# leggedrobotics/delora

Measured on AMD Instinct MI355X. Metric: training scan-pairs/sec, KITTI 64x2048 range images, higher is better.
Workload: dtype f32; 1 GPU; KITTI-shaped 64x2048, batch=8 pairs/GPU, raw scans of ~141k points (ragged, raster order), steps rotate over 8 distinct HBM-resident batches, online normals, ResNet pose CNN (11.9M params, identity-pretrained state), Adam; BASELINE configs[1]; global_batch=8, parallelism=dp1, cnn=fp32, cnn_impl=hip trunk: fp32 MFMA, fused Winograd F(2x2,3x3) + direct implicit GEMM, channels_last=False, hip_graph=False, distinct_batches=8, priming_steps=8

## Files before the change

### delora_amd/csrc/wino_conv_body.h

```cpp
  constexpr int DEAD = STR == 1 ? 3 : (STR == 2 ? 0 : -1);
  constexpr int TR = WN_TILES / TC;
  constexpr int RH = 2 * TR + 2, RW = 2 * TC + 2;
  constexpr int NPIX = RH * RW, NRI = (NPIX + 31) / 32;
  constexpr int RAWBUF = NRI * 256;
  constexpr int NR_IT = (NRI + 7) / 8;
  constexpr int BUF = 2 * 16 * WN_PLANE;
  static_assert((2 * BUF + 2 * RAWBUF) * 4 <= 163840, "LDS budget");
  __shared__ __attribute__((aligned(16))) float lds[2 * BUF + 2 * RAWBUF];
  float* rawbase = lds + 2 * BUF;
#define WN_BUFOF(CH) (lds + (((CH) + 1) & 1) * BUF)

  const int tid = threadIdx.x, lane = tid & 63, wave = __builtin_amdgcn_readfirstlane(tid >> 6);
  const int li = lane & 31, half = lane >> 5;
  const int mb = wave & 1, nb = (wave >> 1) & 1, xh = wave >> 2;
  const int KT = a.K / WN_KB;
  const int tiles_w = RAG ? ((a.W + 1) / 2 + TC - 1) / TC : (a.W / 2) / TC;
  const int tiles_h = RAG ? ((a.H + 1) / 2 + TR - 1) / TR : (a.H / 2) / TR;
  const int nsplit = SPLIT ? a.splits : 1;
  const int ngroups = a.N * tiles_h * tiles_w * KT * nsplit;
  const int nchunks = a.C / WN_CK / nsplit;

  const int tb = wave & 3, tc4 = lane & 1, ttile = (wave >> 2) * 32 + (lane >> 1);
  const int ttr = ttile / TC, ttc = ttile % TC;
  const int j0 = tb == 0 ? 0 : (tb == 2 ? 2 : 1), j1 = tb == 2 ? 1 : (tb == 3 ? 3 : 2);
  const float sgn_s = tb == 1 ? 1.f : -1.f;
  const f32x2 sgn = {sgn_s, sgn_s};
  const int t_wr = tb * WN_PLANE + ttile * 8 + ((tc4 ^ ((ttile >> 3) & 1)) * 4);
  const int t_rd = ((2 * ttr) * RW + 2 * ttc) * 8 + tc4 * 4;
  constexpr int NRAW_W = (NRI + 1) / 2;
  const unsigned lane16 = 16u * (unsigned)lane;
  const int arow = mb * 32 + li, brow = nb * 32 + li;
  const int a_off = arow * 8 + ((half ^ ((arow >> 3) & 1)) * 4);
  const int b_off = 16 * WN_PLANE + brow * 8 + ((half ^ ((brow >> 3) & 1)) * 4);

  int n, k0, gh, gw;
  int cb = 0;
  float* ysp = a.y;
  const float* xn;
  int rowmask[4];
  bool edge;
  unsigned raw_g[NR_IT];
#define WN_SETUP(G, LN)                                                                                                   \
  {                                                                                                                       \
    int t_ = wn_xcd_swizzle((G), ngroups);                                                                                \
    if (SPLIT) { cb = (t_ % nsplit) * nchunks; t_ /= nsplit; }        \
    const int kt_ = t_ % KT; t_ /= KT;                                                                                    \
    gw = t_ % tiles_w; t_ /= tiles_w;                                                                                     \
    gh = t_ % tiles_h;                                                                                                    \
    n = t_ / tiles_h;                                                                                                     \
    k0 = kt_ * WN_KB;                                                                                                     \
    const int h_base_ = gh * TR * 2 - 1, w_base_ = gw * TC * 2 - 1;                       \
    xn = a.x + (size_t)n * a.H * a.W * a.C;                                                                               \
    _Pragma("unroll") for (int i = 0; i < 4; ++i) {                                                                       \
      const int h_ = h_base_ + 2 * ttr + i;                                                                               \
      rowmask[i] = (h_ >= 0 && h_ < a.H) ? -1 : 0;                                                                        \
    }                                                                                                                     \
    edge = __builtin_amdgcn_readfirstlane((int)(h_base_ < 0 || h_base_ + RH > a.H)) != 0;                                                                           \
    _Pragma("unroll") for (int it = 0; it < NR_IT; ++it) {                                                                \
      const int p_ = min(min(2 * wave + it, NRI - 1) * 32 + ((LN) >> 1), NPIX - 1);         \
      int h_ = h_base_ + p_ / RW;                                                                                         \
      h_ = h_ < 0 ? 0 : (h_ >= a.H ? a.H - 1 : h_);                                                                       \
      int w_ = w_base_ + p_ % RW;                                                                                         \
      if (RAG) { w_ %= a.W; w_ = w_ < 0 ? w_ + a.W : w_; }        \
      else w_ = w_ < 0 ? w_ + a.W : (w_ >= a.W ? w_ - a.W : w_);                                                           \
      raw_g[it] = 4u * (unsigned)((h_ * a.W + w_) * a.C + ((LN) & 1) * 4);                                       \
    }                                                                                                                     \
  }

  const unsigned lds_base = (unsigned)(__SIZE_TYPE__)((__attribute__((address_space(3))) char*)lds);
  const int m0_raw = __builtin_amdgcn_readfirstlane((int)(lds_base + 4u * (unsigned)(2 * BUF + min(2 * wave, NRI - 1) * 256)));
  const int m0_u = __builtin_amdgcn_readfirstlane((int)(lds_base + 4u * (unsigned)(16 * WN_PLANE + 2 * wave * WN_PLANE)));
#define WN_RAW_ALL(CH)                                                                                                    \
  {                                                                                                                       \
    const float* rp_ = xn + ((CH) + cb) * WN_CK;                                                                          \
    const int m_ = m0_raw + ((CH) & 1) * (RAWBUF * 4);                                                                    \
    if (2 * wave + 1 < NRI)                                                                                               \
      asm volatile("s_mov_b32 m0, %0\n\ts_nop 0\n\tglobal_load_lds_dwordx4 %1, %3\n\tglobal_load_lds_dwordx4 %2, %4 offset:1024"     \
                   :: "s"(m_), "v"(raw_g[0]), "v"(raw_g[NR_IT - 1]), "s"(rp_), "s"(rp_ - 256) : "memory");                  \
    else if (2 * wave < NRI)                                                                                              \
      asm volatile("s_mov_b32 m0, %0\n\ts_nop 0\n\tglobal_load_lds_dwordx4 %1, %2" :: "s"(m_), "v"(raw_g[0]), "s"(rp_) : "memory");  \
  }
#define WN_U_ALL(CH, BUFP)                                                                                                \
  {                                                                                                                       \
    const float* up_ = a.u + (((size_t)((CH) + cb) * KT + (k0 >> 6)) * 16 + 2 * wave) * 512;                               \
    const int m_ = m0_u + (int)((BUFP) - lds) * 4;                                                                        \
    if (DEAD == 3 && (wave & 1))                                                 \
      asm volatile("s_mov_b32 m0, %0\n\ts_nop 0\n\tglobal_load_lds_dwordx4 %1, %2\n\tglobal_load_lds_dwordx4 %1, %2 offset:1024" \
                   :: "s"(m_), "v"(lane16), "s"(up_) : "memory");                                                         \
    else if (DEAD == 0 && !(wave & 1))                                                           \
      asm volatile("s_mov_b32 m0, %0\n\ts_nop 0\n\tglobal_load_lds_dwordx4 %1, %2 offset:2112\n\tglobal_load_lds_dwordx4 %1, %2 offset:3136" \
                   :: "s"(m_), "v"(lane16), "s"(up_ - 16) : "memory");                                                    \
    else                                                                                                                  \
    asm volatile("s_mov_b32 m0, %0\n\ts_nop 0\n\tglobal_load_lds_dwordx4 %1, %2\n\tglobal_load_lds_dwordx4 %1, %2 offset:1024\n\t" \
                 "global_load_lds_dwordx4 %1, %3 offset:2112\n\tglobal_load_lds_dwordx4 %1, %3 offset:3136"                \
                 :: "s"(m_), "v"(lane16), "s"(up_), "s"(up_ - 16) : "memory");                                            \
  }
#define WN_TROW_LD(I, RB)                                                                                                 \
  {                                                                                                                       \
    dd[(I) & 1][0] = *reinterpret_cast<const i32x4*>((RB) + t_rd + ((I) * RW + j0) * 8);                                  \
    dd[(I) & 1][1] = *reinterpret_cast<const i32x4*>((RB) + t_rd + ((I) * RW + j1) * 8);                                  \
  }
#define WN_TROW_FIN(I)                                                                                                    \
  {                                                                                                                       \
    if (edge) { asm volatile("" ::: "memory"); dd[(I) & 1][0] &= rowmask[I]; dd[(I) & 1][1] &= rowmask[I]; }      \
    const f32x4 da_ = __builtin_bit_cast(f32x4, dd[(I) & 1][0]), db_ = __builtin_bit_cast(f32x4, dd[(I) & 1][1]);         \
    asm volatile("v_pk_fma_f32 %0, %1, %2, %3" : "=v"(tt[I][0]) : "v"(__builtin_shufflevector(db_, db_, 0, 1)), "s"(sgn), "v"(__builtin_shufflevector(da_, da_, 0, 1))); \
    asm volatile("v_pk_fma_f32 %0, %1, %2, %3" : "=v"(tt[I][1]) : "v"(__builtin_shufflevector(db_, db_, 2, 3)), "s"(sgn), "v"(__builtin_shufflevector(da_, da_, 2, 3))); \
  }
#define WN_TROW(I, RB) WN_TROW_LD(I, RB) WN_TROW_FIN(I)
#define WN_PK_ADD(X, Y) ({ f32x2 l_, h_;                                                                                    \
    asm volatile("v_pk_add_f32 %0, %1, %2" : "=v"(l_) : "v"((X)[0]), "v"((Y)[0]));                                        \
    asm volatile("v_pk_add_f32 %0, %1, %2" : "=v"(h_) : "v"((X)[1]), "v"((Y)[1]));                                        \
    __builtin_shufflevector(l_, h_, 0, 1, 2, 3); })
#define WN_PK_SUB(X, Y) ({ f32x2 l_, h_;                                                                                    \
    asm volatile("v_pk_add_f32 %0, %1, %2 neg_lo:[0,1] neg_hi:[0,1]" : "=v"(l_) : "v"((X)[0]), "v"((Y)[0]));              \
    asm volatile("v_pk_add_f32 %0, %1, %2 neg_lo:[0,1] neg_hi:[0,1]" : "=v"(h_) : "v"((X)[1]), "v"((Y)[1]));              \
    __builtin_shufflevector(l_, h_, 0, 1, 2, 3); })
#define WN_V0()                                                                                                           \
  {                                                                                                                       \
    f32x2 tt[4][2];                                                                                                       \
    i32x4 dd[2][2];                                                                                                       \
    const float* rb_ = rawbase;                                                                                           \
    float* vb_ = WN_BUFOF(0) + t_wr;                                                                                      \
    WN_TROW(0, rb_) WN_TROW(1, rb_) WN_TROW(2, rb_) WN_TROW(3, rb_)                                                       \
    *reinterpret_cast<f32x4*>(vb_ + 0 * 4 * WN_PLANE) = WN_PK_SUB(tt[0], tt[2]);                                                    \
    *reinterpret_cast<f32x4*>(vb_ + 1 * 4 * WN_PLANE) = WN_PK_ADD(tt[1], tt[2]);                                                    \
    *reinterpret_cast<f32x4*>(vb_ + 2 * 4 * WN_PLANE) = WN_PK_SUB(tt[2], tt[1]);                                                    \
    *reinterpret_cast<f32x4*>(vb_ + 3 * 4 * WN_PLANE) = WN_PK_SUB(tt[1], tt[3]);                                                    \
  }
#define WN_LOAD_FRAGS_FROM(XL, BP)                                                                                        \
  {                                                                                                                       \
    av[(XL) & 1] = *reinterpret_cast<const f32x4*>((BP) + (xh * 8 + (XL)) * WN_PLANE + a_off);                            \
    bv[(XL) & 1] = *reinterpret_cast<const f32x4*>((BP) + (xh * 8 + (XL)) * WN_PLANE + b_off);                            \
  }
#define WN_LOAD_FRAGS(XL) WN_LOAD_FRAGS_FROM(XL, cur)
#define WN_M(XL, J, ...)                                                                                                  \
  {                                                                                                                       \
    acc[XL] = __builtin_amdgcn_mfma_f32_32x32x2f32(av[(XL) & 1][J], bv[(XL) & 1][J], acc[XL], 0, 0, 0);                   \
    __VA_ARGS__                                                                                                           \
    __builtin_amdgcn_sched_barrier(0);                                                                                    \
  }
#define WN_MZ(XL, J, ...)                                                                                                 \
  {                                                                                                                       \
    acc[XL] = __builtin_amdgcn_mfma_f32_32x32x2f32(av[(XL) & 1][J], bv[(XL) & 1][J], wn_zero16, 0, 0, 0);                 \
    __VA_ARGS__                                                                                                           \
    __builtin_amdgcn_sched_barrier(0);                                                                                    \
  }
#define WN_LOAD_FRAGS_B(XL, B, BP)                                                                                        \
  {                                                                                                                       \
    av[B] = *reinterpret_cast<const f32x4*>((BP) + (xh * 8 + (XL)) * WN_PLANE + a_off);                                   \
    bv[B] = *reinterpret_cast<const f32x4*>((BP) + (xh * 8 + (XL)) * WN_PLANE + b_off);                                   \
  }
#define WN_MB(XL, B, J, ...)                                                                                              \
  {                                                                                                                       \
    acc[XL] = __builtin_amdgcn_mfma_f32_32x32x2f32(av[B][J], bv[B][J], acc[XL], 0, 0, 0);                                 \
    __VA_ARGS__                                                                                                           \
    __builtin_amdgcn_sched_barrier(0);                                                                                    \
  }
#define WN_MZB(XL, B, J, ...)                                                                                             \
  {                                                                                                                       \
    acc[XL] = __builtin_amdgcn_mfma_f32_32x32x2f32(av[B][J], bv[B][J], wn_zero16, 0, 0, 0);                               \
    __VA_ARGS__                                                                                                           \
    __builtin_amdgcn_sched_barrier(0);                                                                                    \
  }

  const f32x16 wn_zero16 = {0.f, 0.f, 0.f, 0.f, 0.f, 0.f, 0.f, 0.f, 0.f, 0.f, 0.f, 0.f, 0.f, 0.f, 0.f, 0.f};
  int grp = blockIdx.x;
  WN_SETUP(grp, lane)
  WN_RAW_ALL(0)
  WN_RAW_ALL(min(1, nchunks - 1))
  WN_U_ALL(0, WN_BUFOF(0))
  asm volatile("s_waitcnt vmcnt(0)" ::: "memory");
  __syncthreads();
  WN_V0()
  for (;;) {
    __syncthreads();
    WN_T(0)
    f32x4 av[2], bv[2];
    f32x2 tt[4][2];
    i32x4 dd[2][2];
    f32x16 acc[8];
    {
      float* cur = WN_BUFOF(0);
      if (DEAD == 0) WN_LOAD_FRAGS_B(1, 0, cur)
      else WN_LOAD_FRAGS(0)
    }
#define WN_CHUNK_BODY(MF)                                                                                                 \
    {                                                                                                                     \
      float* cur = WN_BUFOF(ch);                                                                                          \
      float* nxt = WN_BUFOF(ch + 1);                                                                                      \
      const float* rb = rawbase + ((ch + 1) & 1) * RAWBUF;                                                                \
      float* vb = nxt + t_wr;                                                                                             \
      MF(0, 0, WN_IF_FR(WN_LOAD_FRAGS(1))) WN_M(0, 1, WN_IF_U(WN_U_ALL(ch + 1, nxt)))                                     \
      WN_M(0, 2, )                                                                                                        \
                            \
      WN_M(0, 3, WN_IF_RAW(if (ch + 2 < nchunks) WN_RAW_ALL(ch + 2)))                                                     \
       \
      MF(1, 0, WN_IF_FR(WN_LOAD_FRAGS(2))) WN_M(1, 1, WN_IF_T(WN_TROW_LD(0, rb) WN_TROW_LD(1, rb))) WN_M(1, 2, ) WN_M(1, 3, WN_IF_T(WN_TROW_FIN(0) WN_TROW_FIN(1))) \
      MF(2, 0, WN_IF_FR(WN_LOAD_FRAGS(3))) WN_M(2, 1, WN_IF_T(WN_TROW_LD(2, rb) WN_TROW_LD(3, rb))) WN_M(2, 2, ) WN_M(2, 3, WN_IF_T(WN_TROW_FIN(2) WN_TROW_FIN(3))) \
      MF(3, 0, WN_IF_FR(WN_LOAD_FRAGS(4)) WN_IF_T(*reinterpret_cast<f32x4*>(vb + 0 * 4 * WN_PLANE) = WN_PK_SUB(tt[0], tt[2]);))   \
      WN_M(3, 1, WN_IF_T(*reinterpret_cast<f32x4*>(vb + 1 * 4 * WN_PLANE) = WN_PK_ADD(tt[1], tt[2]);)) WN_M(3, 2, ) WN_M(3, 3, ) \
      MF(4, 0, WN_IF_FR(WN_LOAD_FRAGS(5)) WN_IF_T(*reinterpret_cast<f32x4*>(vb + 2 * 4 * WN_PLANE) = WN_PK_SUB(tt[2], tt[1]);))   \
      WN_M(4, 1, WN_IF_T(*reinterpret_cast<f32x4*>(vb + 3 * 4 * WN_PLANE) = WN_PK_SUB(tt[1], tt[3]);)) WN_M(4, 2, ) WN_M(4, 3, ) \
      MF(5, 0, WN_IF_FR(WN_LOAD_FRAGS(6))) WN_M(5, 1, ) WN_M(5, 2, ) WN_M(5, 3, )                                         \
      MF(6, 0, WN_IF_FR(WN_LOAD_FRAGS(7))) WN_M(6, 1, ) WN_M(6, 2, ) WN_M(6, 3, )                                         \
      asm volatile("s_waitcnt vmcnt(0) lgkmcnt(0)" ::: "memory");                                                         \
      WN_IF_BAR(__builtin_amdgcn_s_barrier();)                                                                            \
      __builtin_amdgcn_sched_barrier(0);                                                                                  \
      MF(7, 0, WN_IF_FR(WN_LOAD_FRAGS_FROM(0, nxt))) WN_M(7, 1, ) WN_M(7, 2, ) WN_M(7, 3, )                               \
    }
#define WN_TAIL_BODY(MF)                                                                                                  \
    {                                                                                                                     \
      float* cur = WN_BUFOF(nchunks - 1);                                                                                 \
      MF(0, 0, WN_LOAD_FRAGS(1)) WN_M(0, 1, ) WN_M(0, 2, ) WN_M(0, 3, )                                                   \
      MF(1, 0, WN_LOAD_FRAGS(2)) WN_M(1, 1, ) WN_M(1, 2, ) WN_M(1, 3, )                                                   \
      MF(2, 0, WN_LOAD_FRAGS(3)) WN_M(2, 1, ) WN_M(2, 2, ) WN_M(2, 3, )                                                   \
      MF(3, 0, WN_LOAD_FRAGS(4)) WN_M(3, 1, ) WN_M(3, 2, ) WN_M(3, 3, )                                                   \
      MF(4, 0, WN_LOAD_FRAGS(5)) WN_M(4, 1, ) WN_M(4, 2, ) WN_M(4, 3, )                                                   \
      MF(5, 0, WN_LOAD_FRAGS(6)) WN_M(5, 1, ) WN_M(5, 2, ) WN_M(5, 3, )                                                   \
      MF(6, 0, WN_LOAD_FRAGS(7)) WN_M(6, 1, ) WN_M(6, 2, ) WN_M(6, 3, )                                                   \
      MF(7, 0, ) WN_M(7, 1, ) WN_M(7, 2, ) WN_M(7, 3, )                                                                   \
    }
#define WN_TX(...) { __VA_ARGS__ }
#define WN_VST(I, EXPR) WN_TX(*reinterpret_cast<f32x4*>(vb + (I) * 4 * WN_PLANE) = EXPR;)
#define WN_CHUNK_BODY_F(MF)                                                                                               \
    {                                                                                                                     \
      float* cur = WN_BUFOF(ch);                                                                                          \
      float* nxt = WN_BUFOF(ch + 1);                                                                                      \
      const float* rb = rawbase + ((ch + 1) & 1) * RAWBUF;                                                                \
      float* vb = nxt + t_wr;                                                                                             \
      MF(0, 0, 0, WN_LOAD_FRAGS_B(1, 1, cur)) WN_MB(0, 0, 1, WN_U_ALL(ch + 1, nxt)) WN_MB(0, 0, 2, )                      \
      WN_MB(0, 0, 3, if (ch + 2 < nchunks) WN_RAW_ALL(ch + 2))                                                            \
      MF(1, 1, 0, WN_LOAD_FRAGS_B(2, 0, cur)) WN_MB(1, 1, 1, WN_TX(WN_TROW_LD(0, rb) WN_TROW_LD(1, rb))) WN_MB(1, 1, 2, ) \
      WN_MB(1, 1, 3, WN_TX(WN_TROW_FIN(0) WN_TROW_FIN(1)))                                                                \
      MF(2, 0, 0, WN_LOAD_FRAGS_B(4, 1, cur)) WN_MB(2, 0, 1, WN_TX(WN_TROW_LD(2, rb) WN_TROW_LD(3, rb))) WN_MB(2, 0, 2, ) \
      WN_MB(2, 0, 3, WN_TX(WN_TROW_FIN(2) WN_TROW_FIN(3)))                                                                \
      MF(4, 1, 0, WN_LOAD_FRAGS_B(5, 0, cur) WN_VST(0, WN_PK_SUB(tt[0], tt[2])))                                          \
      WN_MB(4, 1, 1, WN_VST(1, WN_PK_ADD(tt[1], tt[2]))) WN_MB(4, 1, 2, ) WN_MB(4, 1, 3, )                                \
      MF(5, 0, 0, WN_LOAD_FRAGS_B(6, 1, cur) WN_VST(2, WN_PK_SUB(tt[2], tt[1])))                                          \
      WN_MB(5, 0, 1, WN_VST(3, WN_PK_SUB(tt[1], tt[3]))) WN_MB(5, 0, 2, ) WN_MB(5, 0, 3, )                                \
      asm volatile("s_waitcnt vmcnt(0) lgkmcnt(0)" ::: "memory");                                                         \
      __builtin_amdgcn_s_barrier();                                                                                       \
      __builtin_amdgcn_sched_barrier(0);                                                                                  \
      MF(6, 1, 0, WN_LOAD_FRAGS_B(0, 0, nxt)) WN_MB(6, 1, 1, ) WN_MB(6, 1, 2, ) WN_MB(6, 1, 3, )                          \
    }
#define WN_TAIL_BODY_F(MF)                                                                                                \
    {                                                                                                                     \
      float* cur = WN_BUFOF(nchunks - 1);                                                                                 \
      MF(0, 0, 0, WN_LOAD_FRAGS_B(1, 1, cur)) WN_MB(0, 0, 1, ) WN_MB(0, 0, 2, ) WN_MB(0, 0, 3, )                          \
      MF(1, 1, 0, WN_LOAD_FRAGS_B(2, 0, cur)) WN_MB(1, 1, 1, ) WN_MB(1, 1, 2, ) WN_MB(1, 1, 3, )                          \
      MF(2, 0, 0, WN_LOAD_FRAGS_B(4, 1, cur)) WN_MB(2, 0, 1, ) WN_MB(2, 0, 2, ) WN_MB(2, 0, 3, )                          \
      MF(4, 1, 0, WN_LOAD_FRAGS_B(5, 0, cur)) WN_MB(4, 1, 1, ) WN_MB(4, 1, 2, ) WN_MB(4, 1, 3, )                          \
      MF(5, 0, 0, WN_LOAD_FRAGS_B(6, 1, cur)) WN_MB(5, 0, 1, ) WN_MB(5, 0, 2, ) WN_MB(5, 0, 3, )                          \
      MF(6, 1, 0, ) WN_MB(6, 1, 1, ) WN_MB(6, 1, 2, ) WN_MB(6, 1, 3, )                                                    \
    }
#define WN_CHUNK_BODY_B(MF)                                                                                               \
    {                                                                                                                     \
      float* cur = WN_BUFOF(ch);                                                                                          \
      float* nxt = WN_BUFOF(ch + 1);                                                                                      \
      const float* rb = rawbase + ((ch + 1) & 1) * RAWBUF;                                                                \
      float* vb = nxt + t_wr;                                                                                             \
      MF(1, 0, 0, WN_LOAD_FRAGS_B(2, 1, cur) WN_U_ALL(ch + 1, nxt))                                                       \
      WN_MB(1, 0, 1, WN_TX(WN_TROW_LD(0, rb) WN_TROW_LD(1, rb)))                                                          \
      WN_MB(1, 0, 2, if (ch + 2 < nchunks) WN_RAW_ALL(ch + 2)) WN_MB(1, 0, 3, WN_TX(WN_TROW_FIN(0) WN_TROW_FIN(1)))       \
      MF(2, 1, 0, WN_LOAD_FRAGS_B(3, 0, cur)) WN_MB(2, 1, 1, WN_TX(WN_TROW_LD(2, rb) WN_TROW_LD(3, rb))) WN_MB(2, 1, 2, ) \
      WN_MB(2, 1, 3, WN_TX(WN_TROW_FIN(2) WN_TROW_FIN(3)))                                                                \
      MF(3, 0, 0, WN_LOAD_FRAGS_B(5, 1, cur) WN_VST(0, WN_PK_SUB(tt[0], tt[2])))                                          \
      WN_MB(3, 0, 1, WN_VST(1, WN_PK_ADD(tt[1], tt[2]))) WN_MB(3, 0, 2, ) WN_MB(3, 0, 3, )                                \
      MF(5, 1, 0, WN_LOAD_FRAGS_B(6, 0, cur) WN_VST(2, WN_PK_SUB(tt[2], tt[1])))                                          \
      WN_MB(5, 1, 1, WN_VST(3, WN_PK_SUB(tt[1], tt[3]))) WN_MB(5, 1, 2, ) WN_MB(5, 1, 3, )                                \
      MF(6, 0, 0, WN_LOAD_FRAGS_B(7, 1, cur)) WN_MB(6, 0, 1, ) WN_MB(6, 0, 2, ) WN_MB(6, 0, 3, )                          \
      asm volatile("s_waitcnt vmcnt(0) lgkmcnt(0)" ::: "memory");                                                         \
      __builtin_amdgcn_s_barrier();                                                                                       \
      __builtin_amdgcn_sched_barrier(0);                                                                                  \
      MF(7, 1, 0, WN_LOAD_FRAGS_B(1, 0, nxt)) WN_MB(7, 1, 1, ) WN_MB(7, 1, 2, ) WN_MB(7, 1, 3, )                          \
    }
#define WN_TAIL_BODY_B(MF)                                                                                                \
    {                                                                                                                     \
      float* cur = WN_BUFOF(nchunks - 1);                                                                                 \
      MF(1, 0, 0, WN_LOAD_FRAGS_B(2, 1, cur)) WN_MB(1, 0, 1, ) WN_MB(1, 0, 2, ) WN_MB(1, 0, 3, )                          \
      MF(2, 1, 0, WN_LOAD_FRAGS_B(3, 0, cur)) WN_MB(2, 1, 1, ) WN_MB(2, 1, 2, ) WN_MB(2, 1, 3, )                          \
      MF(3, 0, 0, WN_LOAD_FRAGS_B(5, 1, cur)) WN_MB(3, 0, 1, ) WN_MB(3, 0, 2, ) WN_MB(3, 0, 3, )                          \
      MF(5, 1, 0, WN_LOAD_FRAGS_B(6, 0, cur)) WN_MB(5, 1, 1, ) WN_MB(5, 1, 2, ) WN_MB(5, 1, 3, )                          \
      MF(6, 0, 0, WN_LOAD_FRAGS_B(7, 1, cur)) WN_MB(6, 0, 1, ) WN_MB(6, 0, 2, ) WN_MB(6, 0, 3, )                          \
      MF(7, 1, 0, ) WN_MB(7, 1, 1, ) WN_MB(7, 1, 2, ) WN_MB(7, 1, 3, )                                                    \
    }
    if (DEAD == 3) {
      if (nchunks > 1) {
        { const int ch = 0; WN_CHUNK_BODY_F(WN_MZB) }
        for (int ch = 1; ch + 1 < nchunks; ++ch) WN_CHUNK_BODY_F(WN_MB)
        WN_TAIL_BODY_F(WN_MB)
      } else WN_TAIL_BODY_F(WN_MZB)
    } else if (DEAD == 0) {
      if (nchunks > 1) {
        { const int ch = 0; WN_CHUNK_BODY_B(WN_MZB) }
        for (int ch = 1; ch + 1 < nchunks; ++ch) WN_CHUNK_BODY_B(WN_MB)
        WN_TAIL_BODY_B(WN_MB)
      } else WN_TAIL_BODY_B(WN_MZB)
    } else
    if (nchunks > 1) {
      { const int ch = 0; WN_CHUNK_BODY(WN_MZ) }
      for (int ch = 1; ch + 1 < nchunks; ++ch) WN_CHUNK_BODY(WN_M)
      WN_TAIL_BODY(WN_M)
    } else WN_TAIL_BODY(WN_MZ)
#undef WN_CHUNK_BODY
#undef WN_TAIL_BODY
#undef WN_CHUNK_BODY_F
#undef WN_TAIL_BODY_F
#undef WN_CHUNK_BODY_B
#undef WN_TAIL_BODY_B
#undef WN_TX
#undef WN_VST
    __syncthreads();
    WN_T(1)

    int lane_e = lane;
    asm volatile("" : "+v"(lane_e));
    const int li_e = lane_e & 31, half_e = lane_e >> 5;
    unsigned ooff[8];
    {
      const int lcol = (lane_e >> 4) * 2 + ((lane_e >> 3) & 1);
      const unsigned lane_off = (unsigned)(lcol * a.K + (lane_e & 7) * 4);
#pragma unroll
      for (int it = 0; it < 8; ++it) {
        const int ut = 4 * (mb * 8 + it), tr = ut / TC, tc = ut % TC;
        const int oh = (gh * TR + tr) * 2 + xh, ow0 = (gw * TC + tc) * 2;
        ooff[it] = (unsigned)(((n * a.H + oh) * a.W + ow0) * a.K + k0 + nb * 32) + lane_off;
        if (RAG && (oh >= a.H || ow0 + lcol >= a.W)) ooff[it] = 0xffffffffu;
      }
    }
    unsigned goff[8];
    bool grid_block = true;
    if (STR == 2) {
      const int kh = a.K >> 1;
      const int lcol = (lane_e >> 4) * 2 + ((lane_e >> 3) & 1);
      grid_block = k0 < kh;
#pragma unroll
      for (int it = 0; it < 8; ++it) {
        const int ut = 4 * (mb * 8 + it), tr = ut / TC, tc = ut % TC;
        const int oh = (gh * TR + tr) * 2 + xh, ow0 = (gw * TC + tc) * 2;
        goff[it] = grid_block ? (unsigned)(((n * a.H + oh) * a.W + ow0 + lcol) * kh + k0 + nb * 32 + (lane_e & 7) * 4) : 0u;
      }
    }
    const unsigned (&aoff)[8] = STR == 2 ? goff : ooff;
    if (SPLIT) ysp = a.y + (size_t)(cb / nchunks) * ((size_t)a.N * a.H * a.W * a.K);
    const int nextg = grp + gridDim.x;
    const bool more = nextg < ngroups;
    if (more) {
      WN_SETUP(nextg, lane_e)
      WN_RAW_ALL(0)
      WN_RAW_ALL(min(1, nchunks - 1))
      WN_U_ALL(0, WN_BUFOF(0))
    }

    f32x16 keep[2];
    float* xch = lds;
    const int blk = wave & 3;
    {
      float* dst = xch + ((blk * 2 + xh) * 32) * 64 + lane_e;
#pragma unroll
      for (int q = 0; q < 2; ++q) {
        f32x16 p0, p1;
        if (DEAD == 0) {
          if (q == 0) { p0 = acc[1] + acc[2]; p1 = acc[5] + acc[6]; }
          else        { p0 = wn_sub16(wn_sub16(acc[1], acc[2]), acc[3]); p1 = wn_sub16(wn_sub16(acc[5], acc[6]), acc[7]); }
        } else if (DEAD == 3) {
          if (q == 0) { p0 = acc[0] + acc[1] + acc[2]; p1 = acc[4] + acc[5] + acc[6]; }
          else        { p0 = wn_sub16(acc[1], acc[2]); p1 = wn_sub16(acc[5], acc[6]); }
        } else
        if (q == 0) { p0 = acc[0] + acc[1] + acc[2]; p1 = acc[4] + acc[5] + acc[6]; }
        else        { p0 = wn_sub16(wn_sub16(acc[1], acc[2]), acc[3]); p1 = wn_sub16(wn_sub16(acc[5], acc[6]), acc[7]); }
        f32x16 snd;
        if (xh == 0) { keep[q] = p0 + p1; snd = p1; }
        else         { keep[q] = wn_nsub16(p0, p1); snd = p0; }
#pragma unroll
        for (int r = 0; r < 16; ++r) dst[(q * 16 + r) * 64] = snd[r];
        __builtin_amdgcn_sched_barrier(0);
      }
    }
    const bool f_add = (a.epi & WN_EPI_ADD) && (STR != 2 || grid_block), f_act = a.epi & WN_EPI_ACT, f_dact = a.epi & WN_EPI_DACT;
    __syncthreads();
    {
      const float* src = xch + ((blk * 2 + (xh ^ 1)) * 32) * 64 + lane_e;
#pragma unroll
      for (int q = 0; q < 2; ++q)
#pragma unroll
        for (int r = 0; r < 16; ++r) keep[q][r] += src[(q * 16 + r) * 64];
    }
    __syncthreads();
    WN_T(2)
    constexpr int ES = 32;
    static_assert(8 * 64 * ES <= BUF, "the transposition space must stay inside the lower (V, U) buffer");
    float* ep = lds + wave * (64 * ES);
#pragma unroll
    for (int q = 0; q < 2; ++q)
#pragma unroll
      for (int r = 0; r < 16; ++r) ep[(((r & 3) + 8 * (r >> 2) + 4 * half_e) * 2 + q) * ES + li_e] = keep[q][r];
    f32x4 opv[8];
    {
      const bool has_op = f_dact || f_add;
      const float* op = f_dact ? a.dsrc : (f_add ? a.add : a.u);
#pragma unroll
      for (int it = 0; it < 8; ++it) opv[it] = *reinterpret_cast<const f32x4*>(op + ((has_op && (!RAG || ooff[it] != 0xffffffffu)) ? (STR == 2 && !f_dact ? goff[it] : ooff[it]) : 0u));
    }
    if (more) {
      asm volatile("s_waitcnt vmcnt(0) lgkmcnt(0)" ::: "memory");
      __builtin_amdgcn_s_barrier();
      __builtin_amdgcn_sched_barrier(0);
      WN_V0()
    }
    WN_T(3)
    const bool tanh_act = a.act == 1;
    if (tanh_act || !(f_act || f_dact)) {
      const float* epl = ep + (lane_e >> 3) * ES + (lane_e & 7) * 4;
      if (f_dact) { if (f_add) wn_store_items<true, false, true, RAG>(epl, opv, ooff, aoff, ysp, a.add); else wn_store_items<false, false, true, RAG>(epl, opv, ooff, aoff, ysp, a.add); }
      else if (f_act) { if (f_add) wn_store_items<true, true, false, RAG>(epl, opv, ooff, aoff, ysp, a.add); else wn_store_items<false, true, false, RAG>(epl, opv, ooff, aoff, ysp, a.add); }
      else { if (f_add) wn_store_items<true, false, false, RAG>(epl, opv, ooff, aoff, ysp, a.add); else wn_store_items<false, false, false, RAG>(epl, opv, ooff, aoff, ysp, a.add); }
    } else
#pragma unroll
    for (int it = 0; it < 8; ++it) {
      const int i = lane_e + it * 64, row = i >> 3, c4 = i & 7;
      if (RAG && ooff[it] == 0xffffffffu) continue;
      f32x4 v = *reinterpret_cast<const f32x4*>(ep + row * ES + c4 * 4);
      if (f_add) v += f_dact ? *reinterpret_cast<const f32x4*>(a.add + aoff[it]) : opv[it];
      if (f_act) {
        if (tanh_act) { v[0] = dl_tanh(v[0]); v[1] = dl_tanh(v[1]); v[2] = dl_tanh(v[2]); v[3] = dl_tanh(v[3]); }
        else { v[0] = wn_act(v[0], a.act); v[1] = wn_act(v[1], a.act); v[2] = wn_act(v[2], a.act); v[3] = wn_act(v[3], a.act); }
      }
      if (f_dact) {
        const f32x4 sv = opv[it];
        if (tanh_act) v *= 1.f - sv * sv;
        else { v[0] *= wn_dact(sv[0], a.act); v[1] *= wn_dact(sv[1], a.act); v[2] *= wn_dact(sv[2], a.act); v[3] *= wn_dact(sv[3], a.act); }
      }
      *reinterpret_cast<f32x4*>(ysp + ooff[it]) = v;
    }
    WN_T(4)
    if (!more) break;
    grp = nextg;
  }
#undef WN_BUFOF
#undef WN_SETUP
#undef WN_RAW_ALL
#undef WN_U_ALL
#undef WN_TROW
#undef WN_PK_ADD
#undef WN_PK_SUB
#undef WN_TROW_LD
#undef WN_TROW_FIN
#undef WN_V0
#undef WN_LOAD_FRAGS
#undef WN_LOAD_FRAGS_FROM
#undef WN_M
#undef WN_MZ
#undef WN_LOAD_FRAGS_B
#undef WN_MB
#undef WN_MZB
```

Before: 688.9 scan-pairs/s.

## Skip dead Winograd tiles in stride-2 conv and rotate persistent group walk

Adds a reduced transform-tile schedule (WN_CHUNK_BODY_E) that loads only half of the U filter fragments and skips the MFMAs for tiles known to be dead. Stride-2 blocks in the grid half of K and part of the stride-1 chunk range use it, and the skipped accumulators are zeroed. It also changes how persistent blocks walk groups in the stride-2 path, rotating the group index per round to spread work, presumably for load balance or cache locality. The cost being removed is wasted matrix FLOPs and filter loads. The risk is correctness: the DEAD==3 path now splits chunks into halves without the nchunks>1 guard.

```diff
diff --git a/delora_amd/csrc/wino_conv_body.h b/delora_amd/csrc/wino_conv_body.h
--- a/delora_amd/csrc/wino_conv_body.h
+++ b/delora_amd/csrc/wino_conv_body.h
@@ -95,6 +95,22 @@
                  "global_load_lds_dwordx4 %1, %3 offset:2112\n\tglobal_load_lds_dwordx4 %1, %3 offset:3136"                \
                  :: "s"(m_), "v"(lane16), "s"(up_), "s"(up_ - 16) : "memory");                                            \
   }
+#define WN_U_EV(CH, BUFP)                                                                                                 \
+  {                                                                                                                       \
+    const float* up_ = a.u + (((size_t)((CH) + cb) * KT + (k0 >> 6)) * 16 + 2 * wave) * 512;                               \
+    const int m_ = m0_u + (int)((BUFP) - lds) * 4;                                                                        \
+    if (wave & 1)                                                                                                         \
+      asm volatile("s_mov_b32 m0, %0\n\ts_nop 0\n\tglobal_load_lds_dwordx4 %1, %2\n\tglobal_load_lds_dwordx4 %1, %2 offset:1024" \
+                   :: "s"(m_), "v"(lane16), "s"(up_) : "memory");                                                         \
+    else                                                                                                                  \
+      asm volatile("s_mov_b32 m0, %0\n\ts_nop 0\n\tglobal_load_lds_dwordx4 %1, %2 offset:2112\n\tglobal_load_lds_dwordx4 %1, %2 offset:3136" \
+                   :: "s"(m_), "v"(lane16), "s"(up_ - 16) : "memory");                                                    \
+  }
+#define WN_U_FIRST()                                                                                                      \
+  {                                                                                                                       \
+    if (STR == 1 || (STR == 2 && k0 < (a.K >> 1))) WN_U_EV(0, WN_BUFOF(0))                                                \
+    else WN_U_ALL(0, WN_BUFOF(0))                                                                                         \
+  }
 #define WN_TROW_LD(I, RB)                                                                                                 \
   {                                                                                                                       \
     dd[(I) & 1][0] = *reinterpret_cast<const i32x4*>((RB) + t_rd + ((I) * RW + j0) * 8);                                  \
@@ -166,10 +182,12 @@
 
   const f32x16 wn_zero16 = {0.f, 0.f, 0.f, 0.f, 0.f, 0.f, 0.f, 0.f, 0.f, 0.f, 0.f, 0.f, 0.f, 0.f, 0.f, 0.f};
   int grp = blockIdx.x;
+  int rnd = 0;
+#define WN_WALK(R) ((R) * (int)gridDim.x + (((R) + 1) * (int)gridDim.x <= ngroups ? (int)((blockIdx.x + (unsigned)((R) * 4 * KT)) % gridDim.x) : (int)blockIdx.x))
   WN_SETUP(grp, lane)
   WN_RAW_ALL(0)
   WN_RAW_ALL(min(1, nchunks - 1))
-  WN_U_ALL(0, WN_BUFOF(0))
+  WN_U_FIRST()
   asm volatile("s_waitcnt vmcnt(0)" ::: "memory");
   __syncthreads();
   WN_V0()
@@ -182,7 +200,7 @@
     f32x16 acc[8];
     {
       float* cur = WN_BUFOF(0);
-      if (DEAD == 0) WN_LOAD_FRAGS_B(1, 0, cur)
+      if (STR != 0) WN_LOAD_FRAGS_B(1, 0, cur)
       else WN_LOAD_FRAGS(0)
     }
 #define WN_CHUNK_BODY(MF)                                                                                                 \
@@ -223,19 +241,46 @@
     }
 #define WN_TX(...) { __VA_ARGS__ }
 #define WN_VST(I, EXPR) WN_TX(*reinterpret_cast<f32x4*>(vb + (I) * 4 * WN_PLANE) = EXPR;)
-#define WN_CHUNK_BODY_F(MF)                                                                                               \
+#define WN_CHUNK_BODY_E(MF, UA, NX)                                                                                       \
     {                                                                                                                     \
       float* cur = WN_BUFOF(ch);                                                                                          \
       float* nxt = WN_BUFOF(ch + 1);                                                                                      \
       const float* rb = rawbase + ((ch + 1) & 1) * RAWBUF;                                                                \
       float* vb = nxt + t_wr;                                                                                             \
-      MF(0, 0, 0, WN_LOAD_FRAGS_B(1, 1, cur)) WN_MB(0, 0, 1, WN_U_ALL(ch + 1, nxt)) WN_MB(0, 0, 2, )                      \
+      MF(1, 0, 0, WN_LOAD_FRAGS_B(2, 1, cur) UA(ch + 1, nxt))                                                             \
+      WN_MB(1, 0, 1, WN_TX(WN_TROW_LD(0, rb) WN_TROW_LD(1, rb)))                                                          \
+      WN_MB(1, 0, 2, if (ch + 2 < nchunks) WN_RAW_ALL(ch + 2)) WN_MB(1, 0, 3, WN_TX(WN_TROW_FIN(0) WN_TROW_FIN(1)))       \
+      MF(2, 1, 0, WN_LOAD_FRAGS_B(5, 0, cur)) WN_MB(2, 1, 1, WN_TX(WN_TROW_LD(2, rb) WN_TROW_LD(3, rb))) WN_MB(2, 1, 2, ) \
+      WN_MB(2, 1, 3, WN_TX(WN_TROW_FIN(2) WN_TROW_FIN(3)))                                                                \
+      MF(5, 0, 0, WN_LOAD_FRAGS_B(6, 1, cur) WN_VST(0, WN_PK_SUB(tt[0], tt[2])))                                          \
+      WN_MB(5, 0, 1, WN_VST(1, WN_PK_ADD(tt[1], tt[2]))) WN_MB(5, 0, 2, WN_VST(2, WN_PK_SUB(tt[2], tt[1])))               \
+      WN_MB(5, 0, 3, WN_VST(3, WN_PK_SUB(tt[1], tt[3])))                                                                  \
+      asm volatile("s_waitcnt vmcnt(0) lgkmcnt(0)" ::: "memory");                                                         \
+      __builtin_amdgcn_s_barrier();                                                                                       \
+      __builtin_amdgcn_sched_barrier(0);                                                                                  \
+      MF(6, 1, 0, WN_LOAD_FRAGS_B(NX, 0, nxt)) WN_MB(6, 1, 1, ) WN_MB(6, 1, 2, ) WN_MB(6, 1, 3, )                         \
+    }
+#define WN_TAIL_BODY_E(MF)                                                                                                \
+    {                                                                                                                     \
+      float* cur = WN_BUFOF(nchunks - 1);                                                                                 \
+      MF(1, 0, 0, WN_LOAD_FRAGS_B(2, 1, cur)) WN_MB(1, 0, 1, ) WN_MB(1, 0, 2, ) WN_MB(1, 0, 3, )                          \
+      MF(2, 1, 0, WN_LOAD_FRAGS_B(5, 0, cur)) WN_MB(2, 1, 1, ) WN_MB(2, 1, 2, ) WN_MB(2, 1, 3, )                          \
+      MF(5, 0, 0, WN_LOAD_FRAGS_B(6, 1, cur)) WN_MB(5, 0, 1, ) WN_MB(5, 0, 2, ) WN_MB(5, 0, 3, )                          \
+      MF(6, 1, 0, ) WN_MB(6, 1, 1, ) WN_MB(6, 1, 2, ) WN_MB(6, 1, 3, )                                                    \
+    }
+#define WN_CHUNK_BODY_F(MF0, MF)                                                                                          \
+    {                                                                                                                     \
+      float* cur = WN_BUFOF(ch);                                                                                          \
+      float* nxt = WN_BUFOF(ch + 1);                                                                                      \
+      const float* rb = rawbase + ((ch + 1) & 1) * RAWBUF;                                                                \
+      float* vb = nxt + t_wr;                                                                                             \
+      MF0(0, 0, 0, WN_LOAD_FRAGS_B(1, 1, cur)) WN_MB(0, 0, 1, WN_U_ALL(ch + 1, nxt)) WN_MB(0, 0, 2, )                     \
       WN_MB(0, 0, 3, if (ch + 2 < nchunks) WN_RAW_ALL(ch + 2))                                                            \
       MF(1, 1, 0, WN_LOAD_FRAGS_B(2, 0, cur)) WN_MB(1, 1, 1, WN_TX(WN_TROW_LD(0, rb) WN_TROW_LD(1, rb))) WN_MB(1, 1, 2, ) \
       WN_MB(1, 1, 3, WN_TX(WN_TROW_FIN(0) WN_TROW_FIN(1)))                                                                \
       MF(2, 0, 0, WN_LOAD_FRAGS_B(4, 1, cur)) WN_MB(2, 0, 1, WN_TX(WN_TROW_LD(2, rb) WN_TROW_LD(3, rb))) WN_MB(2, 0, 2, ) \
       WN_MB(2, 0, 3, WN_TX(WN_TROW_FIN(2) WN_TROW_FIN(3)))                                                                \
-      MF(4, 1, 0, WN_LOAD_FRAGS_B(5, 0, cur) WN_VST(0, WN_PK_SUB(tt[0], tt[2])))                                          \
+      MF0(4, 1, 0, WN_LOAD_FRAGS_B(5, 0, cur) WN_VST(0, WN_PK_SUB(tt[0], tt[2])))                                         \
       WN_MB(4, 1, 1, WN_VST(1, WN_PK_ADD(tt[1], tt[2]))) WN_MB(4, 1, 2, ) WN_MB(4, 1, 3, )                                \
       MF(5, 0, 0, WN_LOAD_FRAGS_B(6, 1, cur) WN_VST(2, WN_PK_SUB(tt[2], tt[1])))                                          \
       WN_MB(5, 0, 1, WN_VST(3, WN_PK_SUB(tt[1], tt[3]))) WN_MB(5, 0, 2, ) WN_MB(5, 0, 3, )                                \
@@ -286,17 +331,25 @@
       MF(7, 1, 0, ) WN_MB(7, 1, 1, ) WN_MB(7, 1, 2, ) WN_MB(7, 1, 3, )                                                    \
     }
     if (DEAD == 3) {
-      if (nchunks > 1) {
-        { const int ch = 0; WN_CHUNK_BODY_F(WN_MZB) }
-        for (int ch = 1; ch + 1 < nchunks; ++ch) WN_CHUNK_BODY_F(WN_MB)
-        WN_TAIL_BODY_F(WN_MB)
-      } else WN_TAIL_BODY_F(WN_MZB)
+      const int hc = nchunks >> 1;
+      { const int ch = 0; WN_CHUNK_BODY_E(WN_MZB, WN_U_EV, 1) }
+      for (int ch = 1; ch + 1 < hc; ++ch) WN_CHUNK_BODY_E(WN_MB, WN_U_EV, 1)
+      { const int ch = hc - 1; WN_CHUNK_BODY_E(WN_MB, WN_U_ALL, 0) }
+      { const int ch = hc; WN_CHUNK_BODY_F(WN_MZB, WN_MB) }
+      for (int ch = hc + 1; ch + 1 < nchunks; ++ch) WN_CHUNK_BODY_F(WN_MB, WN_MB)
+      WN_TAIL_BODY_F(WN_MB)
     } else if (DEAD == 0) {
-      if (nchunks > 1) {
+      if (k0 < (a.K >> 1)) {
+        { const int ch = 0; WN_CHUNK_BODY_E(WN_MZB, WN_U_EV, 1) }
+        for (int ch = 1; ch + 1 < nchunks; ++ch) WN_CHUNK_BODY_E(WN_MB, WN_U_EV, 1)
+        WN_TAIL_BODY_E(WN_MB)
+        acc[3] = wn_zero16;
+        acc[7] = wn_zero16;
+      } else {
         { const int ch = 0; WN_CHUNK_BODY_B(WN_MZB) }
         for (int ch = 1; ch + 1 < nchunks; ++ch) WN_CHUNK_BODY_B(WN_MB)
         WN_TAIL_BODY_B(WN_MB)
-      } else WN_TAIL_BODY_B(WN_MZB)
+      }
     } else
     if (nchunks > 1) {
       { const int ch = 0; WN_CHUNK_BODY(WN_MZ) }
@@ -305,6 +358,8 @@
     } else WN_TAIL_BODY(WN_MZ)
 #undef WN_CHUNK_BODY
 #undef WN_TAIL_BODY
+#undef WN_CHUNK_BODY_E
+#undef WN_TAIL_BODY_E
 #undef WN_CHUNK_BODY_F
 #undef WN_TAIL_BODY_F
 #undef WN_CHUNK_BODY_B
@@ -344,13 +399,13 @@
     }
     const unsigned (&aoff)[8] = STR == 2 ? goff : ooff;
     if (SPLIT) ysp = a.y + (size_t)(cb / nchunks) * ((size_t)a.N * a.H * a.W * a.K);
-    const int nextg = grp + gridDim.x;
-    const bool more = nextg < ngroups;
+    const int nextg = STR == 2 ? WN_WALK(rnd + 1) : grp + gridDim.x;
+    const bool more = STR == 2 ? (rnd + 1) * (int)gridDim.x + (int)blockIdx.x < ngroups : nextg < ngroups;
     if (more) {
       WN_SETUP(nextg, lane_e)
       WN_RAW_ALL(0)
       WN_RAW_ALL(min(1, nchunks - 1))
-      WN_U_ALL(0, WN_BUFOF(0))
+      WN_U_FIRST()
     }
 
     f32x16 keep[2];
@@ -437,11 +492,15 @@
     WN_T(4)
     if (!more) break;
     grp = nextg;
-  }
+    ++rnd;
+  }
+#undef WN_WALK
 #undef WN_BUFOF
 #undef WN_SETUP
 #undef WN_RAW_ALL
 #undef WN_U_ALL
+#undef WN_U_EV
+#undef WN_U_FIRST
 #undef WN_TROW
 #undef WN_PK_ADD
 #undef WN_PK_SUB
```

Measured after the change: 693.2 scan-pairs/s, median of 6. Within noise of the previous version (+0.6%).
